# prashantraina/neural_raytracing

Measured on AMD Instinct MI355X. Metric: ray-samples/sec/GPU (800x800x64, 8x256 MLP); PSNR vs ref, higher is better.
Workload: dtype fp32; 1 GPU; 800x800 NeRFCamera frame per GPU, 64 march steps + 130-eval coarse scan per ray, SDF MLP 8x256 F16, 8x NeuralBSDF(6x96) + 16x256 spatial MLP + LightField(10x256, output x10), NeRFIntegrator(Direct); samples_per_ray=64, parallelism=row-tile shard x1 (10-row tiles) + RCCL all-gather

## Files before the change

neural_raytracing_amd/csrc/nrt_common.hip:

```cpp
#include "nrt_launch.h"

#include <atomic>
#include <vector>

namespace nrt {

static thread_local std::string g_err;

void set_error(const std::string& msg) { g_err = msg; }

int hip_fail(hipError_t e, const char* what) {
  g_err = std::string(what) + ": " + hipGetErrorString(e);
  return NRT_EHIP;
}

int max_hidden(const nrt_mlp* m) { return m ? m->desc.hidden : 0; }

struct OptionDef {
  const char* name;
  int64_t def;
};
static const OptionDef kOptions[OPT_COUNT] = {
    {"ring16", 1}, {"ring32", 1}, {"normals16", 1}, {"scan_best32", 1},
    {"march_blocks", 0}, {"shade_program", 1}, {"nerf_fused", 1}, {"max_waves", 0},
    {"shade_ring", 1}, {"normals_ring", 1}, {"xcd_lines", 0},
    {"mixed_refine_d", kMixedRefineD}, {"mixed_refine_s", kMixedRefineS}, {"mixed_restart", 1},
    {"mixed_drift", 0}, {"ring_occlusion", 1}, {"mixed_zone", 500000},
    {"bwd_colsplit", 1}, {"bwd_ring", 1}, {"march_queue", 2}, {"train_save", 1}, {"wgrad_tile", 0},
    {"march_stage", 1}, {"prim_march", 1}, {"scan_saturate", 1},
};
static std::atomic<int64_t> g_opts[OPT_COUNT] = {1, 1, 1, 1, 0, 1, 1, 0, 1, 1, 0,
                                                 kMixedRefineD, kMixedRefineS, 1, 0, 1, 500000, 1, 1, 2, 1, 0,
                                                 1, 1, 1};

int64_t option(Option o) { return g_opts[o].load(std::memory_order_relaxed); }

static int option_index(const char* name) {
  if (!name) return -1;
  for (int i = 0; i < OPT_COUNT; ++i)
    if (std::strcmp(kOptions[i].name, name) == 0) return i;
  return -1;
}

struct ProfRec {
  std::string name;
  hipEvent_t a, b;
  double flop;
};
static bool g_prof = false;
static bool g_prof_evals = false;
static std::vector<ProfRec> g_recs;

ProfScope::ProfScope(const char* n, hipStream_t s, double f) : name(n), stream(s), flop(f) {
  if (!g_prof) return;
  if (hipEventCreate(&start) != hipSuccess) { start = nullptr; return; }
  (void)hipEventRecord(start, stream);
}

ProfScope::~ProfScope() {
  if (!start) return;
  hipEvent_t stop;
  if (hipEventCreate(&stop) != hipSuccess) return;
  (void)hipEventRecord(stop, stream);
  g_recs.push_back({name, start, stop, flop});
}

static unsigned long long* g_evals[64] = {};
static uint64_t g_staged = 0;

void profile_count_staged() {
  if (g_prof_evals) ++g_staged;
}

unsigned long long* profile_eval_counter() {
  if (!g_prof_evals) return nullptr;
  int dev = 0;
  if (hipGetDevice(&dev) != hipSuccess || dev < 0 || dev >= 64) return nullptr;
  if (!g_evals[dev]) {
    if (hipMalloc(&g_evals[dev], 2 * sizeof(unsigned long long)) != hipSuccess) { g_evals[dev] = nullptr; return nullptr; }
    if (hipMemset(g_evals[dev], 0, 2 * sizeof(unsigned long long)) != hipSuccess) return nullptr;
  }
  return g_evals[dev];
}

}

using namespace nrt;

extern "C" {

void nrt_profile_enable(int flags) {
  nrt::g_prof = (flags & NRT_PROF_TIMING) != 0;
  nrt::g_prof_evals = (flags & NRT_PROF_EVALS) != 0;
  if (nrt::g_prof_evals) (void)nrt::profile_eval_counter();
}

void nrt_profile_reset(void) {
  for (auto& r : nrt::g_recs) { (void)hipEventDestroy(r.a); (void)hipEventDestroy(r.b); }
  nrt::g_recs.clear();
  nrt::g_staged = 0;
  int dev = 0;
  if (hipGetDevice(&dev) == hipSuccess && dev >= 0 && dev < 64 && nrt::g_evals[dev])
    (void)hipMemset(nrt::g_evals[dev], 0, 2 * sizeof(unsigned long long));
}

int nrt_profile_evals(uint64_t* evals) {
  if (!evals) { set_error("nrt_profile_evals: null argument"); return NRT_EINVAL; }
  *evals = 0;
  int dev = 0;
  NRT_HIP(hipGetDevice(&dev));
  if (dev < 0 || dev >= 64 || !nrt::g_evals[dev]) return NRT_OK;
  unsigned long long v = 0;
  NRT_HIP(hipMemcpy(&v, nrt::g_evals[dev], sizeof(v), hipMemcpyDeviceToHost));
  *evals = v;
  return NRT_OK;
}
// ... 77 lines not shown
```

neural_raytracing_amd/csrc/nrt_device.h:

```cpp
#pragma once
#include <hip/hip_runtime.h>
#include <stdint.h>

#include <utility>

namespace nrt {

typedef _Float16 h8 __attribute__((ext_vector_type(8)));
typedef float f16v __attribute__((ext_vector_type(16)));

#define NRT_GLOBAL __attribute__((address_space(1)))
#define NRT_CONST __attribute__((address_space(4)))

constexpr int kMaxLin = 20;

#ifndef NRT_RING_RB
#define NRT_RING_RB 2
#endif
constexpr int kRingRB = NRT_RING_RB;

enum { ACT_LEAKY = 0, ACT_SOFTPLUS = 1, ACT_NONE = 2, ACT_SIGMOID = 3, ACT_RELU = 4 };

struct MlpDev {
  int in_size, hidden, n_hidden, out, freqs, skip, latent, act;
// ... 1192 lines not shown
            const h8 b = enc_frag_k<ACT>(basis, s, NE - 1, h, x0, x1, x2);
#pragma unroll
            for (int ib = 0; ib < NB; ++ib) acc[ib] = mfma16(A[(j * NB + ib) * 64], b, acc[ib]);
          }
        }
        E.end();
      }
    }
  }
  kact<NB, ACT>(acc, hv);
  f16v o = E.bias_at(pm, pm.L + 1, 0, h);
  {
    const h8* A = E.begin();
#pragma unroll
    for (int s = 0; s < 2 * NB; ++s) o = mfma16(A[s * 64], hv[s], o);
    E.end();
  }
  return o;
}

__device__ __forceinline__ float tile_row(const f16v& o, int j, int lane) {
  const int reg = (j & 3) + 4 * (j >> 3), hh = (j >> 2) & 1;
  return __shfl(o[reg], (lane & 31) + 32 * hh);
}

}

namespace ring32 {

typedef float f4v __attribute__((ext_vector_type(4)));

__device__ __forceinline__ f4v mfma4(float a, float b, f4v c) {
  return __builtin_amdgcn_mfma_f32_16x16x4f32(a, b, c, 0, 0, 0);
}

constexpr int kSub = 4;

constexpr int kPair32F4 = 7;
__host__ __device__ inline int sphere_pairs32(int n) { return ((n + 3) / 4 + 1) / 2; }
__device__ __forceinline__ void build_sphere_pairs32(const SdfDev& s, float4* out) {
  const int n = s.n_spheres, R = 4 * sphere_pairs32(n);
  const float4* src = reinterpret_cast<const float4*>(s.spheres);
  for (int rec = threadIdx.x; rec < R; rec += blockDim.x) {
    const int g = rec & 3, j = rec >> 2;
    float* o = reinterpret_cast<float*>(out + rec * kPair32F4);
#pragma unroll
    for (int u = 0; u < 2; ++u) {
      const int i = g + 8 * j + 4 * u;
      if (i < n) {
        const float4 r0 = src[4 * i], r1 = src[4 * i + 1], r2 = src[4 * i + 2], r3 = src[4 * i + 3];
        const float m[13] = {r0.x, r0.y, r0.z, r0.w, r1.x, r1.y, r1.z, r1.w, r2.x, r2.y, r2.z, r2.w,
                             r3.x};
        for (int k = 0; k < 13; ++k) o[2 * k + u] = m[k];
      } else {
        for (int k = 0; k < 12; ++k) o[2 * k + u] = 0.f;
        o[24 + u] = -__builtin_inff();
      }
    }
    o[26] = 0.f; o[27] = 0.f;
  }
}

template <int KH, int KE, int WV>
struct Engine {
  static constexpr int QH = KH / 4, QE = KE / 4;
  static constexpr int MAXQ = kSub * (QH > QE ? QH : QE);
  static constexpr int MAXL = (MAXQ + WV - 1) / WV;
  static constexpr int SLOTQ = MAXL * WV;
  static constexpr int RING_BYTES = 2 * SLOTQ * 1024;
  static constexpr int kOutOfRange = 0x40000000;
  static size_t lds_bytes(int F, size_t bias_bytes, size_t sphere_bytes) {
    return RING_BYTES + (size_t)F * 16 + bias_bytes + sphere_bytes;
  }
  const float4* ring;
  uint32_t ring_lds;
  const float* lbias;
  const float4* lbasis;
  const float4* lspheres;
  const void* sbase;
  int sbytes, bstride;
  int off, next_off;
  int slot;
  int lane, wv;

  __device__ __forceinline__ void issue(int qoff, int nq, int s) {
    const int w = __builtin_amdgcn_readfirstlane(wv);
    const uint64_t sp = (uint64_t)(uintptr_t)sbase;
    const uint64_t spu = ((uint64_t)(uint32_t)__builtin_amdgcn_readfirstlane((int)(sp >> 32)) << 32) |
                         (uint32_t)__builtin_amdgcn_readfirstlane((int)(uint32_t)sp);
    const __amdgpu_buffer_rsrc_t r = __builtin_amdgcn_make_buffer_rsrc(
        (void*)(uintptr_t)spu, 0, __builtin_amdgcn_readfirstlane(sbytes), 0x00020000);
    const int q0 = __builtin_amdgcn_readfirstlane(qoff) + w;
    const uint32_t dst0 = __builtin_amdgcn_readfirstlane(ring_lds + (uint32_t)(s * SLOTQ * 1024)) +
                          (uint32_t)w * 1024u;
    const int n = __builtin_amdgcn_readfirstlane(nq);
#pragma unroll
    for (int q = 0; q < MAXL; ++q) {
      const bool own = w + WV * q < n;
      ring::lds_dma16(r, own ? lane * 16 : kOutOfRange + lane * 16, (q0 + WV * q) * 1024,
                      dst0 + (uint32_t)(WV * q * 1024));
    }
  }

  __device__ __forceinline__ void init(const MlpDev& m, const SdfDev& s, char* lds, int nq0) {
    ring = reinterpret_cast<const float4*>(lds);
    ring_lds = (uint32_t)(uintptr_t)(__attribute__((address_space(3))) char*)lds;
    char* p = lds + RING_BYTES;
    const int F = m.freqs;
    float4* lq = reinterpret_cast<float4*>(p);
    for (int q = threadIdx.x; q < F; q += blockDim.x)
      lq[q] = make_float4(m.basis[q], m.basis[F + q], m.basis[2 * F + q], 0.f);
    lbasis = lq;
    p += (size_t)F * 16;
    float* lb = reinterpret_cast<float*>(p);
    const int nb = (m.n_hidden + 2) * m.bias16_stride;
    for (int i = threadIdx.x; i < nb; i += blockDim.x) lb[i] = m.bias32[i];
    lbias = lb;
    p += (size_t)nb * 4;
    float4* ls = reinterpret_cast<float4*>(p);
    if (s.kind == 2) build_sphere_pairs32(s, ls);
    lspheres = ls;
    bstride = m.bias16_stride;
    sbase = m.stream32;
    sbytes = m.stream32_bytes;
    lane = threadIdx.x & 63;
    wv = __builtin_amdgcn_readfirstlane(threadIdx.x >> 6);
    off = 0;
    slot = 0;
    issue(0, nq0, 0);
    __syncthreads();
  }
  __device__ __forceinline__ const float4* begin(int nq, int nq_next, bool wrap) {
    asm volatile("" ::: "memory");
    __builtin_amdgcn_s_waitcnt(ring::waitcnt_vm_lgkm0(0));
    __builtin_amdgcn_s_barrier();
    asm volatile("" ::: "memory");
    next_off = wrap ? 0 : off + nq;
    issue(next_off, nq_next, slot ^ 1);
    __builtin_amdgcn_sched_barrier(0);
    return ring + slot * SLOTQ * 64 + lane;
  }
  __device__ __forceinline__ void end() {
    off = next_off;
    slot ^= 1;
  }
  __device__ __forceinline__ void drain() { __builtin_amdgcn_s_waitcnt(ring::waitcnt_vm_lgkm0(0)); }
  __device__ __forceinline__ f4v bias_at(int layer, int sb) const {
    const float4 q = *reinterpret_cast<const float4*>(lbias + layer * bstride + 16 * sb + 4 * (lane >> 4));
    return f4v{q.x, q.y, q.z, q.w};
  }
};

__device__ __forceinline__ float softplus_f32(float x) { return softplus_exact(x); }

template <int ACT>
__device__ __forceinline__ float act(float x) {
  if (ACT == ACT_SOFTPLUS) return softplus_f32(x);
  return act_fwd<false>(x, ACT);
}

template <int NQ, int P0, int BO, int NBV, class Side>
__device__ __forceinline__ void seg2(const float4* A, const float (&B)[NBV], f4v& a0, f4v& a1,
                                     Side&& side) {
  float4 w0 = A[P0 * 64], w1 = A[(P0 + 1) * 64];
#pragma unroll
  for (int u = 0; u < NQ; ++u) {
    side(u);
    float4 n0 = w0, n1 = w1;
    if (u + 1 < NQ) { n0 = A[(P0 + 2 * u + 2) * 64]; n1 = A[(P0 + 2 * u + 3) * 64]; }
    a0 = mfma4(w0.x, B[BO + 4 * u], a0); a1 = mfma4(w1.x, B[BO + 4 * u], a1);
    a0 = mfma4(w0.y, B[BO + 4 * u + 1], a0); a1 = mfma4(w1.y, B[BO + 4 * u + 1], a1);
    a0 = mfma4(w0.z, B[BO + 4 * u + 2], a0); a1 = mfma4(w1.z, B[BO + 4 * u + 2], a1);
    a0 = mfma4(w0.w, B[BO + 4 * u + 3], a0); a1 = mfma4(w1.w, B[BO + 4 * u + 3], a1);
    w0 = n0; w1 = n1;
  }
}
template <int NQ, int P0, int BO, int NBV>
__device__ __forceinline__ void seg2(const float4* A, const float (&B)[NBV], f4v& a0, f4v& a1) {
  seg2<NQ, P0, BO>(A, B, a0, a1, [](int) {});
}

template <int NQ, int P0, int BO, int NBV, class Side>
__device__ __forceinline__ void seg4(const float4* A, const float (&B)[NBV], f4v (&a)[kSub],
                                     Side&& side) {
  float4 w[kSub];
#pragma unroll
  for (int b = 0; b < kSub; ++b) w[b] = A[(P0 + b) * 64];
#pragma unroll
  for (int u = 0; u < NQ; ++u) {
    side(u);
    float4 n[kSub];
#pragma unroll
    for (int b = 0; b < kSub; ++b) n[b] = (u + 1 < NQ) ? A[(P0 + kSub * (u + 1) + b) * 64] : w[b];
#pragma unroll
    for (int b = 0; b < kSub; ++b) a[b] = mfma4(w[b].x, B[BO + 4 * u], a[b]);
#pragma unroll
    for (int b = 0; b < kSub; ++b) a[b] = mfma4(w[b].y, B[BO + 4 * u + 1], a[b]);
#pragma unroll
    for (int b = 0; b < kSub; ++b) a[b] = mfma4(w[b].z, B[BO + 4 * u + 2], a[b]);
#pragma unroll
    for (int b = 0; b < kSub; ++b) a[b] = mfma4(w[b].w, B[BO + 4 * u + 3], a[b]);
#pragma unroll
    for (int b = 0; b < kSub; ++b) w[b] = n[b];
  }
}

template <int ACT>
__device__ __forceinline__ float act_tan32(float z, bool value) {
  const float zv = ring::quad_leader(z);
  return value ? act<ACT>(zv) : act_bwd(zv, ACT) * z;
}

template <int KH, int KE, int WV, int ACT, bool TAN = false>
__device__ __forceinline__ float eval(Engine<KH, KE, WV>& E, const MlpDev& m, float x0, float x1,
                                      float x2) {
  using En = Engine<KH, KE, WV>;
  constexpr int QH = En::QH, QE = En::QE;
  constexpr int NC = KH / (4 * kSub);
  static_assert(QH >= 8 && KH % (4 * kSub) == 0, "hidden chunks must spread the pending activations");
  const int g = E.lane >> 4;
  const int comp = TAN ? (E.lane & 3) : 0;
  const bool value = comp == 0;
  const int F = m.freqs, L = m.n_hidden, SK = m.skip;
  float eraw[KE], eact[KE];
#pragma unroll
  for (int e = 0; e < KE; ++e) {
    const int slot = 4 * e + g;
    float v = 0.f, tv = 0.f;
    if (slot < 2 * F) {
      const float4 b = E.lbasis[slot >> 1];
      float pr = x0 * b.x;
      pr = fmaf(x1, b.y, pr);
      pr = fmaf(x2, b.z, pr);
      float sn, cs;
      sincosf(pr, &sn, &cs);
      v = (slot & 1) ? cs : sn;
      if (TAN) {
        const float bk = comp == 1 ? b.x : comp == 2 ? b.y : b.z;
        tv = (slot & 1) ? -sn * bk : cs * bk;
      }
    } else if (slot == 2 * F) {
      v = x0;
      tv = comp == 1 ? 1.f : 0.f;
    } else if (slot == 2 * F + 1) {
      v = x1;
      tv = comp == 2 ? 1.f : 0.f;
    } else if (slot == 2 * F + 2) {
      v = x2;
      tv = comp == 3 ? 1.f : 0.f;
    }
    if (TAN && !value) {
      eraw[e] = tv;
      eact[e] = act_bwd(v, ACT) * tv;
    } else {
      eraw[e] = v;
      eact[e] = act<ACT>(v);
    }
  }
  const float bmask = value ? 1.f : 0.f;
  auto bias = [&](int layer, int sb) {
    f4v b = E.bias_at(layer, sb);
    if (TAN) b *= bmask;
    return b;
  };
  constexpr int CH = kSub * QH, CE = kSub * QE;
  auto first_q = [&](int i) { return i >= L ? QH : CH; };
  float src[KH], dst[KH];
  f4v pend[kSub];
  auto retire1 = [&](int ib, int k) {
    const int r = k & 3;
    float& d = dst[4 * kSub * ib + k];
    if (TAN) d = act_tan32<ACT>(pend[k >> 2][r], value);
    else d = act<ACT>(pend[k >> 2][r]);
    asm volatile("" : "+v"(d));
  };
  constexpr bool PK = !TAN && ACT == ACT_SOFTPLUS;
  auto retire2 = [&](int ib, int q) {
    if constexpr (PK) {
      const int k = 2 * q, r = k & 3;
      const f2v v = softplus_exact2(f2v{pend[k >> 2][r], pend[k >> 2][r + 1]});
      float& d0 = dst[4 * kSub * ib + k];
      float& d1 = dst[4 * kSub * ib + k + 1];
      d0 = v[0];
      d1 = v[1];
      asm volatile("" : "+v"(d0), "+v"(d1));
    } else {
      retire1(ib, 2 * q);
      retire1(ib, 2 * q + 1);
    }
  };
  auto retire = [&](int ib) {
#pragma unroll
    for (int q = 0; q < 2 * kSub; ++q) retire2(ib, q);
  };
#pragma unroll
  for (int ib = 0; ib < NC; ++ib) {
    const float4* A = E.begin(CE, ib + 1 < NC ? CE : first_q(0), false);
    f4v a[kSub];
#pragma unroll
    for (int b = 0; b < kSub; ++b) a[b] = bias(0, kSub * ib + b);
    if (ib > 0) retire(ib - 1);
    seg4<QE, 0, 0>(A, eraw, a, [](int) {});
#pragma unroll
    for (int b = 0; b < kSub; ++b) pend[b] = a[b];
    E.end();
  }
  retire(NC - 1);
  for (int i = 0; i < L; ++i) {
#pragma unroll
    for (int k = 0; k < KH; ++k) src[k] = dst[k];
    const bool skip = i != L - 1 && i % SK == 0;
#pragma unroll
    for (int ib = 0; ib < NC; ++ib) {
      const int after = ib + 1 < NC ? CH : first_q(i + 1);
      const float4* A = E.begin(CH, skip ? CE : after, false);
      f4v a[kSub];
#pragma unroll
      for (int b = 0; b < kSub; ++b) a[b] = bias(1 + i, kSub * ib + b);
      seg4<QH, 0, 0>(A, src, a, [&](int u) {
        if (ib > 0)
#pragma unroll
          for (int q = (u * 2 * kSub) / QH; q < ((u + 1) * 2 * kSub) / QH; ++q) retire2(ib - 1, q);
      });
      E.end();
      if (skip) {
        const float4* B = E.begin(CE, after, false);
        seg4<QE, 0, 0>(B, eact, a, [](int) {});
        E.end();
      }
#pragma unroll
      for (int b = 0; b < kSub; ++b) pend[b] = a[b];
    }
    retire(NC - 1);
  }
  const float4* A = E.begin(QH, CE, true);
  f4v o0 = bias(L + 1, 0), o1 = f4v{0.f, 0.f, 0.f, 0.f};
  {
    float4 w0 = A[0], w1 = A[64];
#pragma unroll
    for (int u = 0; u < QH; u += 2) {
      float4 n0 = w0, n1 = w1;
      if (u + 2 < QH) { n0 = A[(u + 2) * 64]; n1 = A[(u + 3) * 64]; }
      o0 = mfma4(w0.x, dst[4 * u], o0); o1 = mfma4(w1.x, dst[4 * u + 4], o1);
      o0 = mfma4(w0.y, dst[4 * u + 1], o0); o1 = mfma4(w1.y, dst[4 * u + 5], o1);
      o0 = mfma4(w0.z, dst[4 * u + 2], o0); o1 = mfma4(w1.z, dst[4 * u + 6], o1);
      o0 = mfma4(w0.w, dst[4 * u + 3], o0); o1 = mfma4(w1.w, dst[4 * u + 7], o1);
      w0 = n0; w1 = n1;
    }
  }
  E.end();
  const float o = o0[0] + o1[0];
  return __shfl(o, E.lane & 15);
}

__device__ __forceinline__ float spheres_value16(const SdfDev& s, const float4* sp, int lane,
                                                 float x, float y, float z) {
  const float nk2 = -s.k * 1.4426950408889634f;
  float acc = 0.f;
  for (int i = lane >> 4; i < s.n_spheres; i += 4) {
    const float4 r0 = sp[4 * i], r1 = sp[4 * i + 1], r2 = sp[4 * i + 2], r3 = sp[4 * i + 3];
    const float qx = fmaf(r0.z, z, fmaf(r0.y, y, r0.x * x)) - r2.y;
    const float qy = fmaf(r1.y, z, fmaf(r1.x, y, r0.w * x)) - r2.z;
    const float qz = fmaf(r2.x, z, fmaf(r1.w, y, r1.z * x)) - r2.w;
    const float d = __builtin_amdgcn_sqrtf(qx * qx + qy * qy + qz * qz) - r3.x;
    acc += __builtin_amdgcn_exp2f(d * nk2);
  }
  acc += __shfl_xor(acc, 16);
  acc += __shfl_xor(acc, 32);
  return -logf(fmaxf(acc, 1e-4f)) / s.k;
}

__device__ __forceinline__ float spheres_value16_pairs(const SdfDev& s, const float4* sp, int lane,
                                                       float x, float y, float z) {
  const int g = lane >> 4, NP = sphere_pairs32(s.n_spheres);
  const float nk = -s.k * 1.4426950408889634f;
  const f2v xx = {x, x}, yy = {y, y}, zz = {z, z}, nk2 = {nk, nk};
  f2v acc = {0.f, 0.f};
  for (int j = 0; j < NP; ++j) {
    const float4* q = sp + (4 * j + g) * kPair32F4;
    const float4 a = q[0], b = q[1], c = q[2], d = q[3], e = q[4], f = q[5], h = q[6];
    const f2v m00 = {a.x, a.y}, m01 = {a.z, a.w}, m02 = {b.x, b.y}, m10 = {b.z, b.w};
    const f2v m11 = {c.x, c.y}, m12 = {c.z, c.w}, m20 = {d.x, d.y}, m21 = {d.z, d.w};
    const f2v m22 = {e.x, e.y}, cx = {e.z, e.w}, cy = {f.x, f.y}, cz = {f.z, f.w};
    const f2v r = {h.x, h.y};
    const f2v qx = __builtin_elementwise_fma(m02, zz, __builtin_elementwise_fma(m01, yy, m00 * xx)) - cx;
    const f2v qy = __builtin_elementwise_fma(m12, zz, __builtin_elementwise_fma(m11, yy, m10 * xx)) - cy;
    const f2v qz = __builtin_elementwise_fma(m22, zz, __builtin_elementwise_fma(m21, yy, m20 * xx)) - cz;
    const f2v n2 = (qx * qx + qy * qy) + qz * qz;
    const f2v dd = f2v{__builtin_amdgcn_sqrtf(n2.x), __builtin_amdgcn_sqrtf(n2.y)} - r;
    const f2v t = dd * nk2;
    acc += f2v{__builtin_amdgcn_exp2f(t.x), __builtin_amdgcn_exp2f(t.y)};
  }
  float v = acc.x + acc.y;
  v += __shfl_xor(v, 16);
  v += __shfl_xor(v, 32);
  return -logf(fmaxf(v, 1e-4f)) / s.k;
}

}
}
```

neural_raytracing_amd/csrc/nrt_kernels.h:

```cpp
#pragma once
#include <hip/hip_runtime.h>

#include <algorithm>
#include <cmath>

#include "nrt_internal.h"
#include "nrt_prim.h"
#include "nrt_ring3.h"

namespace nrt {

constexpr int kLdsBytes = 160 * 1024;

template <bool F16, int NB>
__device__ __forceinline__ void mlp_eval(const MlpDev& m, const EncIn& e, float* X, int RS,
                                         float* Y, int ys, float* zs) {
  if (F16) mlp16_forward<NB>(m, e, Y, ys);
  else mlp32_forward<NB>(m, e, X, RS, Y, ys, zs);
  wave_lds_fence();
}

template <bool F16>
__device__ __forceinline__ void mlp_eval_any(const MlpDev& m, const EncIn& e, float* X, int RS,
                                          float* Y, int ys) {
// ... 146 lines not shown
    for (int o = (lane >> 5); o < m.out; o += 2) y[row * m.out + o] = l.Y[r * m.out + o];
}

template <bool F16, int NB>
__global__ void __launch_bounds__(256, F16 ? 2 : 1) k_sdf_eval(const SdfDev* __restrict__ sp,
                                                   const float* __restrict__ p, int64_t M,
                                                   float* __restrict__ out, int RS, int per_wave) {
  extern __shared__ float smem[];
  const SdfDev& s = *sp;
  WaveLds l = wave_lds(smem, per_wave, RS, F16);
  const int lane = lane_id(), r = lane & 31;
  const int64_t row0 = wave_global() * 32;
  if (row0 >= M) return;
  const int64_t row = row0 + r;
  const int64_t rr = row < M ? row : M - 1;
  float v = sdf_value<F16, NB>(s, p[rr * 3], p[rr * 3 + 1], p[rr * 3 + 2], l, RS, nullptr);
  if (row < M && lane < 32) out[row] = v;
}

template <int NB>
__global__ void __launch_bounds__(256) k_sdf_grad(
    const SdfDev* __restrict__ sp, const float* __restrict__ p, const int32_t* __restrict__ index,
    const int32_t* __restrict__ count, int64_t M, float* __restrict__ grad,
    float* __restrict__ n_out, float* __restrict__ p_io, float offset_eps,
    float* __restrict__ zscr, int RS, int per_wave, int64_t zs_per_wave) {
  extern __shared__ float smem[];
  const SdfDev& s = *sp;
  WaveLds l = wave_lds(smem, per_wave, RS, false);
  const int lane = lane_id(), r = lane & 31;
  const int64_t nw = (int64_t)gridDim.x * (blockDim.x >> 6);
  const int64_t gw = wave_global();
  float* zs = zscr ? zscr + gw * zs_per_wave : nullptr;
  const int64_t total = count ? (int64_t)(*count) : M;
  for (int64_t w = gw; w * 32 < total; w += nw) {
    const int64_t i = w * 32 + r;
    const bool valid = i < total;
    const int64_t ii = valid ? i : total - 1;
    const int64_t idx = index ? (int64_t)index[ii] : ii;
    const float* pp = p_io ? p_io : p;
    const float x = pp[idx * 3], y = pp[idx * 3 + 1], z = pp[idx * 3 + 2];
    float g[3];
    sdf_gradient<NB>(s, x, y, z, l, RS, zs, g);
    if (valid && lane < 32) {
      if (grad) { grad[idx * 3] = g[0]; grad[idx * 3 + 1] = g[1]; grad[idx * 3 + 2] = g[2]; }
      if (n_out) {
        float nx = g[0], ny = g[1], nz = g[2];
        normalize3(nx, ny, nz, 1e-6f);
        n_out[idx * 3] = nx; n_out[idx * 3 + 1] = ny; n_out[idx * 3 + 2] = nz;
        if (p_io) {
          p_io[idx * 3] = x + (nx * offset_eps) * 5.f;
          p_io[idx * 3 + 1] = y + (ny * offset_eps) * 5.f;
          p_io[idx * 3 + 2] = z + (nz * offset_eps) * 5.f;
        }
      }
    }
  }
}

struct MarchArgs {
  int max_steps;
  float eps;
  float max_t;
  int primary;
  double step;
  int32_t* scan_idx;
  unsigned long long* evals = nullptr;
  const double* groups = nullptr;
  int64_t group_rays = 1;
  int lds_spheres = 0;
  int xcd_lines = 0;
  float refine_d = 0.f, refine_s = 0.f;
  int drift_model = 0;
  float zone = 0.f;
  unsigned long long* amb = nullptr;
  unsigned long long* keys2 = nullptr;
  unsigned long long* kbest = nullptr;
  const unsigned long long* start = nullptr;
  const int32_t* list = nullptr;
  const int32_t* count = nullptr;
  const float* occ_max_t = nullptr;
  unsigned int* queue = nullptr;
  int stage = 0;
  int sat = 0;
};
constexpr float kScanSat = -0.02f;
constexpr float kSatThr = 20.0f;
#ifndef NRT_QUEUE_CHUNK
#define NRT_QUEUE_CHUNK 16
#endif
#ifndef NRT_QUEUE_TAIL
#define NRT_QUEUE_TAIL 16
#endif
constexpr int kQueueChunk = NRT_QUEUE_CHUNK;
constexpr int kQueueTail = NRT_QUEUE_TAIL;

constexpr int kStageSlots = 8;
constexpr int kStageBytes = kStageSlots * 16 * (4 + 8);
template <class W>
struct LineStage {
  W* data;
  W* out;
  int64_t limit;
  int tag = -1;
  uint32_t msk = 0;
  int lane;
  __device__ __forceinline__ void init(W* d, W* o, int64_t lim, int ln) {
    data = d; out = o; limit = lim; lane = ln;
  }
  __device__ __forceinline__ void flush(int q, int line, uint32_t m) {
    if (lane < 16 && ((m >> lane) & 1u)) out[(int64_t)line * 16 + lane] = data[q * 16 + lane];
    if (lane == q) { tag = -1; msk = 0u; }
  }
  __device__ __forceinline__ void put(uint64_t fin, int64_t ray, W v) {
    while (fin) {
      const int l = __builtin_ctzll(fin);
      fin &= fin - 1;
      const int64_t r = ((int64_t)__builtin_amdgcn_readlane((int)(ray >> 32), l) << 32) |
                        (uint32_t)__builtin_amdgcn_readlane((int)(uint32_t)ray, l);
      const int line = (int)(r >> 4), off = (int)(r & 15);
      const uint64_t own = __ballot(lane < kStageSlots && tag == line);
      int q;
      if (own) {
        q = __builtin_ctzll(own);
      } else {
        const uint64_t fr = __ballot(lane < kStageSlots && tag < 0);
        if (fr) {
          q = __builtin_ctzll(fr);
        } else {
          q = 0;
          flush(0, __builtin_amdgcn_readlane(tag, 0), (uint32_t)__builtin_amdgcn_readlane((int)msk, 0));
        }
        if (lane == q) { tag = line; msk = 0u; }
      }
      asm volatile("" ::: "memory");
      if (lane == l) data[q * 16 + off] = v;
      if (lane == q) msk |= 1u << off;
      const uint32_t m = (uint32_t)__builtin_amdgcn_readlane((int)msk, q);
      const int64_t n = limit - (int64_t)line * 16;
      const uint32_t full = n >= 16 ? 0xffffu : ((1u << (int)n) - 1u);
      asm volatile("" ::: "memory");
      if (m == full) flush(q, line, m);
      asm volatile("" ::: "memory");
    }
  }
  __device__ __forceinline__ void drain() {
#pragma unroll
    for (int q = 0; q < kStageSlots; ++q) {
      const int line = __builtin_amdgcn_readlane(tag, q);
      if (line >= 0) flush(q, line, (uint32_t)__builtin_amdgcn_readlane((int)msk, q));
    }
  }
};

__device__ __forceinline__ double scan_step_of(const MarchArgs& a, int64_t ray) {
  return a.groups ? a.groups[ray / a.group_rays] / 128.0 : a.step;
}

template <bool F16, int NB>
__global__ void __launch_bounds__(256, F16 ? 2 : 1) k_intersect(
    const SdfDev* __restrict__ sp, const float* __restrict__ rays, int64_t P, MarchArgs a,
    float* __restrict__ t_out, uint8_t* __restrict__ hit_out, float* __restrict__ p_out,
    float* __restrict__ n_out, float* __restrict__ rawn_out, float* __restrict__ thr_out,
    int32_t* __restrict__ hit_idx, int32_t* __restrict__ hit_count, int RS, int per_wave) {
  extern __shared__ float smem[];
  const SdfDev& s = *sp;
  WaveLds l = wave_lds(smem, per_wave, RS, F16);
// ... 88 lines not shown
  uint32_t b = __float_as_uint(v + 0.f);
  b = (b & 0x80000000u) ? ~b : (b | 0x80000000u);
  return ((uint64_t)b << 32) | (uint32_t)idx;
}
__device__ __forceinline__ float scan_key_value(uint64_t k) {
  uint32_t b = (uint32_t)(k >> 32);
  b = (b & 0x80000000u) ? (b & 0x7fffffffu) : ~b;
  return __uint_as_float(b);
}

#ifndef NRT_RAY_CHUNK
#define NRT_RAY_CHUNK 1
#endif
constexpr int64_t kRayChunk = NRT_RAY_CHUNK;
constexpr int64_t kLineRays = 32;
constexpr int kXcds = 8;
struct OwnedRays {
  int64_t nw, w, full, R;
  bool lines = false;
  int64_t X = 1, g = 0, Rg = 0, nwg = 1, v = 0;
  __device__ __forceinline__ OwnedRays(int64_t P, int64_t nw_, int64_t w_) : nw(nw_), w(w_) {
    const int64_t rounds = P / (nw * kRayChunk);
    full = rounds * kRayChunk;
    const int64_t rem = P - rounds * nw * kRayChunk;
    R = full + (w < rem ? (rem - 1 - w) / nw + 1 : 0);
  }
  __device__ __forceinline__ OwnedRays(int64_t P, int64_t nw_, int64_t w_, int wv, bool xcd)
      : OwnedRays(P, nw_, w_) {
    if (!xcd) return;
    lines = true;
    const int64_t blocks = nw / wv, b = w / wv;
    X = blocks < kXcds ? blocks : kXcds;
    g = b % X;
    const int64_t gb = (blocks - g + X - 1) / X;
    nwg = gb * wv;
    v = (b / X) * wv + (w % wv);
    const int64_t NL = (P + kLineRays - 1) / kLineRays;
    const int64_t ng = NL > g ? (NL - g + X - 1) / X : 0;
    Rg = ng * kLineRays;
    if (ng > 0 && (NL - 1) % X == g) Rg -= NL * kLineRays - P;
    R = v < Rg ? (Rg - 1 - v) / nwg + 1 : 0;
  }
  __device__ __forceinline__ int64_t ray(int64_t k) const {
    if (lines) {
      const int64_t q = v + k * nwg;
      return (g + X * (q / kLineRays)) * kLineRays + (q % kLineRays);
    }
    if (k < full) return ((k / kRayChunk) * nw + w) * kRayChunk + (k % kRayChunk);
    return (full * nw) + w + (k - full) * nw;
  }
};

template <int NB, int NE, int WV, bool FOLD>
struct RingPol16 {
  static constexpr int RPW = 32, WAVES = WV;
  using Eng = ring::Engine<NB, NE, WV>;
  __device__ __forceinline__ static void init(Eng& E, const SdfDev& s, const MlpDev& m, char* lds,
                                              const MarchArgs& a) {
    E.init(m, lds);
    E.lspheres = nullptr;
    if (s.kind == 2 && a.lds_spheres > 0) {
      float4* ls = reinterpret_cast<float4*>(lds + a.lds_spheres);
      ring::build_sphere_pairs(s, ls);
      __syncthreads();
      E.lspheres = ls;
    }
  }
  __device__ __forceinline__ static float sdf(Eng& E, const SdfDev& s, const MlpDev& m, float x, float y, float z) {
    float d = 0.f;
    if (s.kind == 2)
      d = E.lspheres ? ring::spheres_value_pairs(s, E.lspheres, E.lane, x, y, z)
                     : spheres_value<true>(s, x, y, z);
    return d + ring::eval<NB, NE, WV, FOLD, 8, 3>(E, m, x, y, z);
  }
  __device__ __forceinline__ static void finish(Eng&) {}
  static constexpr bool kGuard = false;
  static constexpr bool kSat = FOLD || NB < 8;
  __device__ __forceinline__ static bool retry(Eng&, bool, float) { return false; }
};
template <int KH, int KE, int WV, int ACT>
struct RingPol32 {
  static constexpr int RPW = 16, WAVES = WV;
  using Eng = ring32::Engine<KH, KE, WV>;
  __device__ __forceinline__ static void init(Eng& E, const SdfDev& s, const MlpDev& m, char* lds,
                                              const MarchArgs&) {
    E.init(m, s, lds, ring32::kSub * Eng::QE);
  }
  __device__ __forceinline__ static float sdf(Eng& E, const SdfDev& s, const MlpDev& m, float x, float y, float z) {
    const float d = (s.kind == 2) ? ring32::spheres_value16_pairs(s, E.lspheres, E.lane, x, y, z) : 0.f;
    return d + ring32::eval<KH, KE, WV, ACT>(E, m, x, y, z);
  }
  __device__ __forceinline__ static float tan(Eng& E, const MlpDev& m, float x, float y, float z) {
    return ring32::eval<KH, KE, WV, ACT, true>(E, m, x, y, z);
  }
  __device__ __forceinline__ static void finish(Eng& E) { E.drain(); }
  static constexpr bool kGuard = false;
  static constexpr bool kSat = true;
  __device__ __forceinline__ static bool retry(Eng&, bool, float) { return false; }
};

template <int KH, int KQ, int WV, int ACT>
struct RingPol3 {
  static constexpr int RPW = 16, WAVES = WV;
  using Eng = ring3::Engine<KH, KQ, WV>;
  __device__ __forceinline__ static void init(Eng& E, const SdfDev& s, const MlpDev& m, char* lds,
                                              const MarchArgs&) {
    E.init(m, s, lds, 4 * KQ, 4 * KQ);
  }
  __device__ __forceinline__ static float sdf(Eng& E, const SdfDev& s, const MlpDev& m, float x, float y, float z) {
    const float d = (s.kind == 2) ? ring32::spheres_value16(s, E.lspheres, E.lane, x, y, z) : 0.f;
#ifndef NRT_NOGUARD_EXP
    if (__builtin_amdgcn_readfirstlane((int)E.guarded))
      return d + ring3::eval<KH, KQ, WV, ACT, false, true>(E, m, x, y, z);
#endif
    return d + ring3::eval<KH, KQ, WV, ACT>(E, m, x, y, z);
  }
  __device__ __forceinline__ static float tan(Eng& E, const MlpDev& m, float x, float y, float z) {
    if (__builtin_amdgcn_readfirstlane((int)E.guarded))
      return ring3::eval<KH, KQ, WV, ACT, true, true>(E, m, x, y, z);
    return ring3::eval<KH, KQ, WV, ACT, true>(E, m, x, y, z);
  }
  __device__ __forceinline__ static void finish(Eng& E) { E.drain(); }
  static constexpr bool kGuard = true;
  static constexpr bool kSat = !(KH == 8 && KQ == 3);
  __device__ __forceinline__ static bool retry(Eng& E, bool active, float v) {
    return ring3::retry(E, active, v);
  }
};

template <class Pol, int MODE, bool MX = false>
__device__ __forceinline__ void march_body(
    const SdfDev s, const MlpDev m, const float* __restrict__ rays, int64_t P, MarchArgs a,
    float* __restrict__ t_out, uint8_t* __restrict__ hit_out, float* __restrict__ p_out,
    float* __restrict__ n_out, float* __restrict__ rawn_out, float* __restrict__ thr_out,
    unsigned long long* __restrict__ keys) {
  extern __shared__ __attribute__((aligned(16))) char smem_c[];
  constexpr int mode = MODE;
  constexpr int RPW = Pol::RPW, WV = Pol::WAVES;
  constexpr uint32_t kRayMask = RPW == 32 ? 0xffffffffu : ((1u << RPW) - 1u);
  const int lane = lane_id(), r = lane & (RPW - 1);
  const int64_t nw = (int64_t)gridDim.x * WV;
  const int64_t w = (int64_t)blockIdx.x * WV + __builtin_amdgcn_readfirstlane(threadIdx.x >> 6);
  const int64_t Pe =
      ((MX || MODE == 3) && a.count)
          ? (int64_t)__builtin_amdgcn_readfirstlane(*(const NRT_GLOBAL int32_t*)a.count)
          : P;
  const OwnedRays own(Pe, nw, w, WV, a.xcd_lines != 0);
  const bool dyn = a.queue != nullptr;
  const int64_t R = dyn ? Pe : own.R;
  const bool scan = mode == 0 && a.primary;
  const int64_t tq = kQueueTail * nw;
  const int64_t T = dyn ? (R < tq ? R : tq)
                        : (kScanSplit < 0 ? R : (R < kScanSplit ? R : (int64_t)kScanSplit));
  const bool alt = MX && mode == 1 && a.keys2 != nullptr;
  const bool sat = !MX && (mode == 1 || (mode == 0 && Pol::kSat)) && a.sat != 0;
  const int64_t J = mode == 0 ? (scan ? R + (sat ? 0 : R - T) + T * kScanSegs : R) : (alt ? 2 * R : R);
  const uint32_t lt = (1u << r) - 1u;
  typename Pol::Eng E;
  Pol::init(E, s, m, smem_c, a);
  int kind = -1;
  int64_t ray = 0;
  float ox = 0.f, oy = 0.f, oz = 0.f, dx = 0.f, dy = 0.f, dz = 0.f;
  float t = 0.f, best = 0.f, second = 0.f;
  double step = a.step;
  int i = 0, j = 0, left = 0, idx = 0, idx2 = 0;
  bool ended = false, hit = false, whole = false;
  unsigned long long ambs = ~0ull;
  float drift = 0.f, dprev = 1.f;
  float mt = 0.f;
  unsigned long long cps = ~0ull;
  int64_t cursor = 0;
  int64_t cend = 0;
  bool dry = false;
// ... 952 lines not shown
```

neural_raytracing_amd/csrc/nrt_launch.h:

```cpp
#pragma once
#include <hip/hip_runtime.h>

#include <algorithm>
#include <cmath>
#include <cstdlib>
#include <cstring>
#include <memory>
#include <string>

#include "nrt_internal.h"
#include "nrt_kernels.h"

namespace nrt {

enum Option {
  OPT_RING16 = 0,
  OPT_RING32,
  OPT_NORMALS16,
  OPT_SCAN_BEST32,
  OPT_MARCH_BLOCKS,
  OPT_SHADE_PROGRAM,
  OPT_NERF_FUSED,
  OPT_MAX_WAVES,
  OPT_SHADE_RING,
  OPT_NORMALS_RING,
  OPT_XCD_LINES,
  OPT_MIXED_D,
  OPT_MIXED_S,
  OPT_MIXED_RESTART,
  OPT_MIXED_DRIFT,
  OPT_RING_OCCLUSION,
  OPT_MIXED_ZONE,
  OPT_BWD_COLSPLIT,
  OPT_BWD_RING,
  OPT_MARCH_QUEUE,
  OPT_TRAIN_SAVE,
  OPT_WGRAD_TILE,
  OPT_MARCH_STAGE,
  OPT_PRIM_MARCH,
  OPT_SCAN_SATURATE,
  OPT_COUNT
};
int64_t option(Option o);

#define NRT_NB_SWITCH(nbv, ...)                               \
  switch (nbv) {                                              \
    case 2: { constexpr int NB = 2; __VA_ARGS__; } break;     \
    case 3: { constexpr int NB = 3; __VA_ARGS__; } break;     \
    case 4: { constexpr int NB = 4; __VA_ARGS__; } break;     \
    case 8: { constexpr int NB = 8; __VA_ARGS__; } break;     \
    default: { constexpr int NB = 1; __VA_ARGS__; } break;    \
  }

static inline int ceil_div64(int64_t a, int64_t b) { return (int)((a + b - 1) / b); }

struct LdsPlan {
  int RS = 1;
  int ys = 1;
  int per_wave = 0;
  int waves = 4;
  size_t bytes = 0;
};

static inline int opt_max_waves() {
  const int64_t v = option(OPT_MAX_WAVES);
  return v >= 1 && v <= 4 ? (int)v : 4;
}

static inline LdsPlan plan_lds(int hidden, int ke, int ys, bool f16, bool with_grad, int max_waves = 4) {
  LdsPlan p;
  max_waves = std::min(max_waves, opt_max_waves());
  p.ys = std::max(ys, 1);
  p.RS = f16 ? 1 : slab_stride(std::max(hidden, 32), std::max(ke, 16), with_grad);
  p.per_wave = wave_lds_floats(p.RS, p.ys, f16);
  int per_wave_bytes = p.per_wave * 4;
  p.waves = std::max(1, std::min(max_waves, kLdsBytes / std::max(per_wave_bytes, 1)));
  p.bytes = (size_t)p.waves * per_wave_bytes;
  return p;
}

static inline void spread_waves(LdsPlan& p) {
  const int per_cu = std::min(8, kLdsBytes / std::max(p.per_wave * 4, 1));
  int b = std::min(p.waves, per_cu);
  while (b > 1 && (per_cu / b) * b < per_cu) --b;
  p.waves = std::max(1, b);
  p.bytes = (size_t)p.waves * p.per_wave * 4;
}

template <typename K>
static inline int set_lds(K kernel, size_t bytes) {
  if (bytes > 64 * 1024) {
    hipError_t e = hipFuncSetAttribute(reinterpret_cast<const void*>(kernel),
                                       hipFuncAttributeMaxDynamicSharedMemorySize, (int)bytes);
    if (e != hipSuccess) return hip_fail(e, "hipFuncSetAttribute(MaxDynamicSharedMemorySize)");
  }
  return NRT_OK;
}

static inline void stage_lds(MarchArgs& a, size_t& lds, int waves) {
  if (!a.queue || option(OPT_MARCH_STAGE) == 0) return;
  const size_t off = (lds + 15) & ~(size_t)15;
  const size_t need = off + (size_t)waves * kStageBytes;
  if (off == 0 || need > 160 * 1024) return;
  a.stage = (int)off;
  lds = need;
}

static inline int check_launch(const char* what) {
  hipError_t e = hipGetLastError();
  if (e != hipSuccess) return hip_fail(e, what);
  return NRT_OK;
}

static inline int sdf_dims(const nrt_sdf* s, int& hidden, int& ke) {
  hidden = 32; ke = 16;
  if (s->mlp) { hidden = s->mlp->desc.hidden; ke = s->mlp->host_dev.ke; }
  return NRT_OK;
}

inline bool ring_supported(const nrt_sdf* s) {
  if (!s->mlp || (s->mlp->refreshed && !s->mlp->ring16_refreshed)) return false;
  const MlpDev& m = s->mlp->host_dev;
  const int ne = m.ke / 16;
// ... 158 lines not shown
```

neural_raytracing_amd/csrc/nrt_ring_march32.hip:

```cpp
#include "nrt_launch.h"

#ifndef NRT_R32_SMALL_WV
#define NRT_R32_SMALL_WV 8
#endif

namespace nrt {

static int ring32_launch(const nrt_sdf* s, const float* rays, int64_t P, const MarchArgs& ma,
                         float* t, uint8_t* hit, float* p, float* n, float* raw_n, float* thr,
                         unsigned long long* keys, hipStream_t st, int which) {
  const MlpDev& md = s->mlp->host_dev;
  const size_t extra = (size_t)md.freqs * 16 + ring32_bias_bytes(s) + ring32_sphere_bytes(s);
  int dev = 0, cus = 0;
  NRT_HIP(hipGetDevice(&dev));
  NRT_HIP(hipDeviceGetAttribute(&cus, hipDeviceAttributeMultiprocessorCount, dev));
  const bool scan = ma.primary != 0;
  if (scan && which == 0) NRT_HIP(hipMemsetAsync(keys, 0xff, (size_t)P * sizeof(unsigned long long), st));
  auto run = [&]<int KH, int KE, int ACT>() -> int {
    constexpr int WV = KH <= 32 ? NRT_R32_SMALL_WV : kRing32Waves;
    auto launch = [&](auto kern, const char* name, bool plain = false) -> int {
      size_t lds = ring32::Engine<KH, KE, WV>::RING_BYTES + extra;
      MarchArgs mb = ma;
      if (plain) stage_lds(mb, lds, WV);
      if (mb.stage) profile_count_staged();
      if (int rc = set_lds(kern, lds)) return rc;
      int per_cu = 0;
      NRT_HIP(hipOccupancyMaxActiveBlocksPerMultiprocessor(&per_cu, kern, 64 * WV, lds));
      const int64_t slots = (int64_t)std::max(per_cu, 1) * std::max(cus, 1);
      int blocks = (int)std::max<int64_t>(1, std::min<int64_t>(slots, ceil_div64(P, 16 * WV)));
      if (const int64_t f = option(OPT_MARCH_BLOCKS)) blocks = (int)std::min<int64_t>(f, 1 << 20);
      if (ma.queue) NRT_HIP(hipMemsetAsync(ma.queue, 0, sizeof(unsigned int), st));
      ProfScope prof(name, st);
      kern<<<dim3(blocks), dim3(64 * WV), lds, st>>>(s->host_dev, md, rays, P, mb, t, hit, nullptr,
                                                     nullptr, nullptr, thr, keys);
      return check_launch(name);
    };
    if (which == 2) return launch(k_occl32<KH, KE, WV, ACT>, "k_occl32");
    if (which == 0)
      if (int rc = launch(k_march32<KH, KE, WV, ACT>, "k_march32", true)) return rc;
    if (scan) return launch(k_scan_best32<KH, KE, WV, ACT>, "k_scan_best32");
    return NRT_OK;
  };
  const bool sp = s->mlp->desc.activation == NRT_ACT_SOFTPLUS;
  int rc = NRT_EINVAL;
#define NRT_R32(H, KEV)                                                                   \
  if (md.hidden == H && md.ke == 4 * KEV)                                                 \
    rc = sp ? run.template operator()<H / 4, KEV, ACT_SOFTPLUS>()                         \
            : run.template operator()<H / 4, KEV, ACT_LEAKY>();                           \
  else
  NRT_R32(256, 12) NRT_R32(256, 20) NRT_R32(128, 12) NRT_R32(128, 20) {
    set_error("FP32 ring engine: unsupported SDF configuration");
    return NRT_EINVAL;
  }
#undef NRT_R32
  return rc;
}

int ring_occlusion32(const nrt_sdf* s, const float* rays, int64_t P, const MarchArgs& ma,
                     uint8_t* visible, hipStream_t st) {
  return ring32_launch(s, rays, P, ma, nullptr, visible, nullptr, nullptr, nullptr, nullptr,
                       nullptr, st, 2);
}

int ring_scan_best32(const nrt_sdf* s, const float* rays, int64_t P, const MarchArgs& ma,
                     float* thr, unsigned long long* keys, hipStream_t st) {
  return ring32_launch(s, rays, P, ma, nullptr, nullptr, nullptr, nullptr, nullptr, thr, keys, st, 1);
}

int ring_march32(const nrt_sdf* s, const float* rays, int64_t P, const MarchArgs& ma, float* t,
                 uint8_t* hit, float* p, float* n, float* raw_n, float* thr, int32_t* idx,
                 int32_t* cnt, unsigned long long* keys, hipStream_t st) {
  if (int rc = ring32_launch(s, rays, P, ma, t, hit, p, n, raw_n, thr, keys, st, 0)) return rc;
  k_march_finish<><<<dim3(std::min<int64_t>(ceil_div64(P, 256), 2048)), dim3(256), 0, st>>>(
      rays, P, t, hit, p, n, raw_n, idx, cnt);
  return check_launch("k_march_finish");
}

}
```

Before: 59.28 million ray-samples/s.

## Stagger ring-buffer weight prefetch for the upper half of waves in FP32 march

Adds a march_stagger option (on by default) that marks the upper half of the waves in a block as 'late'. For those waves, the next weight-slot prefetch is issued partway through the current segment's MMA loop (at u==1) rather than right after the barrier. This spreads global/LDS load bursts across the workgroup so memory traffic overlaps compute instead of all waves issuing at once. It risks reading slot data before the deferred waves have filled it, and it adds branching in the hot evaluation loop.

```diff
diff --git a/neural_raytracing_amd/csrc/nrt_common.hip b/neural_raytracing_amd/csrc/nrt_common.hip
--- a/neural_raytracing_amd/csrc/nrt_common.hip
+++ b/neural_raytracing_amd/csrc/nrt_common.hip
@@ -27,11 +27,11 @@
     {"mixed_refine_d", kMixedRefineD}, {"mixed_refine_s", kMixedRefineS}, {"mixed_restart", 1},
     {"mixed_drift", 0}, {"ring_occlusion", 1}, {"mixed_zone", 500000},
     {"bwd_colsplit", 1}, {"bwd_ring", 1}, {"march_queue", 2}, {"train_save", 1}, {"wgrad_tile", 0},
-    {"march_stage", 1}, {"prim_march", 1}, {"scan_saturate", 1},
+    {"march_stage", 1}, {"prim_march", 1}, {"scan_saturate", 1}, {"march_stagger", 1},
 };
 static std::atomic<int64_t> g_opts[OPT_COUNT] = {1, 1, 1, 1, 0, 1, 1, 0, 1, 1, 0,
                                                  kMixedRefineD, kMixedRefineS, 1, 0, 1, 500000, 1, 1, 2, 1, 0,
-                                                 1, 1, 1};
+                                                 1, 1, 1, 1};
 
 int64_t option(Option o) { return g_opts[o].load(std::memory_order_relaxed); }
 
diff --git a/neural_raytracing_amd/csrc/nrt_device.h b/neural_raytracing_amd/csrc/nrt_device.h
--- a/neural_raytracing_amd/csrc/nrt_device.h
+++ b/neural_raytracing_amd/csrc/nrt_device.h
@@ -1298,6 +1298,8 @@
   int off, next_off;
   int slot;
   int lane, wv;
+  int late = 0;
+  int deferred_nq;
 
   __device__ __forceinline__ void issue(int qoff, int nq, int s) {
     const int w = __builtin_amdgcn_readfirstlane(wv);
@@ -1346,15 +1348,21 @@
     issue(0, nq0, 0);
     __syncthreads();
   }
-  __device__ __forceinline__ const float4* begin(int nq, int nq_next, bool wrap) {
+  __device__ __forceinline__ const float4* begin(int nq, int nq_next, bool wrap,
+                                                 bool defer = false) {
     asm volatile("" ::: "memory");
     __builtin_amdgcn_s_waitcnt(ring::waitcnt_vm_lgkm0(0));
     __builtin_amdgcn_s_barrier();
     asm volatile("" ::: "memory");
     next_off = wrap ? 0 : off + nq;
-    issue(next_off, nq_next, slot ^ 1);
+    deferred_nq = nq_next;
+    if (!defer) issue(next_off, nq_next, slot ^ 1);
     __builtin_amdgcn_sched_barrier(0);
     return ring + slot * SLOTQ * 64 + lane;
+  }
+  __device__ __forceinline__ void issue_deferred() {
+    issue(next_off, deferred_nq, slot ^ 1);
+    __builtin_amdgcn_sched_barrier(0);
   }
   __device__ __forceinline__ void end() {
     off = next_off;
@@ -1427,9 +1435,10 @@
   return value ? act<ACT>(zv) : act_bwd(zv, ACT) * z;
 }
 
-template <int KH, int KE, int WV, int ACT, bool TAN = false>
+template <int KH, int KE, int WV, int ACT, bool TAN = false, bool STG = false>
 __device__ __forceinline__ float eval(Engine<KH, KE, WV>& E, const MlpDev& m, float x0, float x1,
                                       float x2) {
+  static_assert(!(TAN && STG), "the staggered stream is the value evaluation's");
   using En = Engine<KH, KE, WV>;
   constexpr int QH = En::QH, QE = En::QE;
   constexpr int NC = KH / (4 * kSub);
@@ -1438,6 +1447,11 @@
   const int comp = TAN ? (E.lane & 3) : 0;
   const bool value = comp == 0;
   const int F = m.freqs, L = m.n_hidden, SK = m.skip;
+  const bool late = STG && __builtin_amdgcn_readfirstlane(E.late) != 0;
+  auto refill = [&](int u) {
+    if constexpr (STG)
+      if (u == 1 && late) E.issue_deferred();
+  };
   float eraw[KE], eact[KE];
 #pragma unroll
   for (int e = 0; e < KE; ++e) {
@@ -1511,12 +1525,12 @@
   };
 #pragma unroll
   for (int ib = 0; ib < NC; ++ib) {
-    const float4* A = E.begin(CE, ib + 1 < NC ? CE : first_q(0), false);
+    const float4* A = E.begin(CE, ib + 1 < NC ? CE : first_q(0), false, late);
     f4v a[kSub];
 #pragma unroll
     for (int b = 0; b < kSub; ++b) a[b] = bias(0, kSub * ib + b);
     if (ib > 0) retire(ib - 1);
-    seg4<QE, 0, 0>(A, eraw, a, [](int) {});
+    seg4<QE, 0, 0>(A, eraw, a, refill);
 #pragma unroll
     for (int b = 0; b < kSub; ++b) pend[b] = a[b];
     E.end();
@@ -1529,19 +1543,20 @@
 #pragma unroll
     for (int ib = 0; ib < NC; ++ib) {
       const int after = ib + 1 < NC ? CH : first_q(i + 1);
-      const float4* A = E.begin(CH, skip ? CE : after, false);
+      const float4* A = E.begin(CH, skip ? CE : after, false, late);
       f4v a[kSub];
 #pragma unroll
       for (int b = 0; b < kSub; ++b) a[b] = bias(1 + i, kSub * ib + b);
       seg4<QH, 0, 0>(A, src, a, [&](int u) {
+        refill(u);
         if (ib > 0)
 #pragma unroll
           for (int q = (u * 2 * kSub) / QH; q < ((u + 1) * 2 * kSub) / QH; ++q) retire2(ib - 1, q);
       });
       E.end();
       if (skip) {
-        const float4* B = E.begin(CE, after, false);
-        seg4<QE, 0, 0>(B, eact, a, [](int) {});
+        const float4* B = E.begin(CE, after, false, late);
+        seg4<QE, 0, 0>(B, eact, a, refill);
         E.end();
       }
 #pragma unroll
diff --git a/neural_raytracing_amd/csrc/nrt_kernels.h b/neural_raytracing_amd/csrc/nrt_kernels.h
--- a/neural_raytracing_amd/csrc/nrt_kernels.h
+++ b/neural_raytracing_amd/csrc/nrt_kernels.h
@@ -252,6 +252,7 @@
   unsigned int* queue = nullptr;
   int stage = 0;
   int sat = 0;
+  int stagger = 0;
 };
 constexpr float kScanSat = -0.02f;
 constexpr float kSatThr = 20.0f;
@@ -506,13 +507,15 @@
 struct RingPol32 {
   static constexpr int RPW = 16, WAVES = WV;
   using Eng = ring32::Engine<KH, KE, WV>;
+  static constexpr bool kStagger = WV >= 2 && !(KH == 64 && KE == 20);
   __device__ __forceinline__ static void init(Eng& E, const SdfDev& s, const MlpDev& m, char* lds,
-                                              const MarchArgs&) {
+                                              const MarchArgs& a) {
     E.init(m, s, lds, ring32::kSub * Eng::QE);
+    E.late = (kStagger && a.stagger != 0 && E.wv >= WV / 2) ? 1 : 0;
   }
   __device__ __forceinline__ static float sdf(Eng& E, const SdfDev& s, const MlpDev& m, float x, float y, float z) {
     const float d = (s.kind == 2) ? ring32::spheres_value16_pairs(s, E.lspheres, E.lane, x, y, z) : 0.f;
-    return d + ring32::eval<KH, KE, WV, ACT>(E, m, x, y, z);
+    return d + ring32::eval<KH, KE, WV, ACT, false, kStagger>(E, m, x, y, z);
   }
   __device__ __forceinline__ static float tan(Eng& E, const MlpDev& m, float x, float y, float z) {
     return ring32::eval<KH, KE, WV, ACT, true>(E, m, x, y, z);
diff --git a/neural_raytracing_amd/csrc/nrt_launch.h b/neural_raytracing_amd/csrc/nrt_launch.h
--- a/neural_raytracing_amd/csrc/nrt_launch.h
+++ b/neural_raytracing_amd/csrc/nrt_launch.h
@@ -39,6 +39,7 @@
   OPT_MARCH_STAGE,
   OPT_PRIM_MARCH,
   OPT_SCAN_SATURATE,
+  OPT_MARCH_STAGGER,
   OPT_COUNT
 };
 int64_t option(Option o);
diff --git a/neural_raytracing_amd/csrc/nrt_ring_march32.hip b/neural_raytracing_amd/csrc/nrt_ring_march32.hip
--- a/neural_raytracing_amd/csrc/nrt_ring_march32.hip
+++ b/neural_raytracing_amd/csrc/nrt_ring_march32.hip
@@ -21,6 +21,7 @@
     auto launch = [&](auto kern, const char* name, bool plain = false) -> int {
       size_t lds = ring32::Engine<KH, KE, WV>::RING_BYTES + extra;
       MarchArgs mb = ma;
+      mb.stagger = option(OPT_MARCH_STAGGER) != 0 ? 1 : 0;
       if (plain) stage_lds(mb, lds, WV);
       if (mb.stage) profile_count_staged();
       if (int rc = set_lds(kern, lds)) return rc;
```

New measurement: 59.72 million ray-samples/s, median of 6. About the same (+0.7%).
